# Biblbrox/ViT-Spectre-Experiments

Hardware: AMD Instinct MI355X
Metric: images/sec training, Spectre-ViT-S CIFAR-100 bs512 (higher is better)
Workload: dtype bf16; 1 GPU; Spectre-ViT-Small (E512 H16 F768 L4 P4 N65, 100 classes, dropout 0.001), fft mixer, train step fwd+CE+bwd+AdamW, bs 512/GPU; mixer=fft, global_batch=512, parallelism=dp1

## Files before the change

### include/spv.h

```cpp
#ifndef SPV_H
#define SPV_H

#include <stdint.h>

#ifdef __cplusplus
extern "C" {
#endif

#define SPV_F32 0
#define SPV_BF16 1

#define SPV_ABI_VERSION 1

int spv_version(void);
enum {
    SPV_PATH_GEMM_STRIP = 0,
    SPV_PATH_GEMM_STRIP_ACC = 1,
    SPV_PATH_GEMM_TN = 2,
    SPV_PATH_TAIL_LC = 3,
    SPV_PATH_TAIL_UP = 4,
    SPV_PATH_TAIL_LN = 5,
    SPV_PATH_FNET_MFMA = 6,
    SPV_PATH_GATHER_LDS = 7,
    SPV_PATH_GEMM_TN_WIDE = 9,
// ... 142 lines not shown
typedef struct spv_step_ctl {
    double a, b;
    float clip_coef;
    int apply;
    float grad_norm;
    int sched_step;
    int skipped;
    int reserved[7];
} spv_step_ctl;
#define SPV_CTL_SCHEDULE 1
#define SPV_CTL_CLIP 2
#define SPV_CTL_SKIP_NONFINITE 4

int spv_grad_sumsq(const void* table, const int* chunk_tensor, const int* chunk_off, const int* sizes, int nchunks, double* partials,
                   void* stream);

int spv_step_control(const double* partials, int npartials, float* const* step_ptrs, int nsteps, spv_step_ctl* ctl, int flags,
                     int warmup_steps, int total_steps, double eta_min, float max_norm, void* stream);

int spv_adamw_multi_ctl(const void* table, const int* chunk_tensor, const int* chunk_off, const int* sizes, int nchunks, double base_lr,
                        float beta1, float beta2, float one_minus_beta1, float one_minus_beta2, float eps, float weight_decay,
                        const float* step_dev, const spv_step_ctl* ctl, void* stream);

int spv_fwht(const void* x, void* y, const void* residual, int rows, int n_in, int n, int n_out, int mode, int repeat,
             float scale, int dtype, void* stream);

int spv_patchify(const float* img, void* out, int batch, int chans, int height, int width, int patch, int ld,
                 int transposed, int out_dtype, void* stream);
int spv_patchify_u8(const unsigned char* img_hwc, const float* mean, const float* inv_std, void* out, int batch, int chans,
                    int height, int width, int patch, int ld, int transposed, int out_dtype, void* stream);
int spv_embed_posbias(const float* pos, const float* bias, const float* cls, float* out, int patches, int embed, void* stream);
int spv_embed_cls_rows(const float* cls, const float* pos, void* tokens, int batch, int tokens_per_image, int embed,
                       int dtype, void* stream);
int spv_spectral_fold(const float* proj_w, const float* freq_h, const float* freq_w, float* w_full, int embed,
                      int chans, int patch, void* stream);
int spv_spectral_fold_bf16(const float* proj_w, const float* freq_h, const float* freq_w, float* w_full, void* w_full_bf16, int embed,
                           int chans, int patch, void* stream);
int spv_spectral_fold_bwd(const float* dw_full, const float* proj_w, const float* freq_h, const float* freq_w,
                          float* dproj_w, float* dfreq_h, float* dfreq_w, float* scratch, int embed, int chans,
                          int patch, void* stream);
int spv_dropout(const void* x, void* y, int64_t n, float p, uint64_t seed, int dtype, void* stream);
int spv_embed_bwd_groups(int batch);
int spv_embed_bwd(const void* g, const void* gcls, void* dtok, float* partials, float* dpos, float* dbias, float* dcls, int batch,
                  int tokens, int embed, float p_drop, uint64_t seed, int dtype, void* stream);

int spv_attention_fwd(const void* qkv, void* ctx, void* probs, int seqs, int len, int heads, int head_dim, int dtype,
                      float p_drop, uint64_t seed, void* stream);
int spv_attention_bwd(const void* dctx, const void* qkv, const void* probs, void* dscores, void* dqkv, int seqs, int len,
                      int heads, int head_dim, int dtype, float p_drop, uint64_t seed, void* stream);
int spv_attention_row0_fwd(const void* q0, const void* k, const void* v, int ldkv, void* ctx0, float* probs, int batch, int len,
                           int heads, int head_dim, int dtype, float p_drop, uint64_t seed, void* stream);
int spv_attention_row0_bwd(const void* dctx0, const void* q0, const void* k, const void* v, int ldkv, const float* probs, void* dq0,
                           void* dk, void* dv, int ldd, int batch, int len, int heads, int head_dim, int dtype, float p_drop,
                           uint64_t seed, void* stream);

int spv_gelu_fwd(const void* x, void* y, int64_t n, int dtype, void* stream);
int spv_gelu_bwd(const void* dy, const void* x, void* dx, int64_t n, int dtype, void* stream);
int spv_colsum(const void* x, float* out, float* partials, int rows, int n, int dtype, void* stream);
int spv_axpby(const void* x, const void* y, void* out, float a, float b, int64_t n, int dtype, void* stream);

int spv_small_sl_supported(int rows, int n, int k);
int64_t spv_small_sl_partial_floats(int rows, int n);
int spv_small_sl_fwd(const void* xa, int64_t lda, const void* xb, int64_t ldb, const float* W, const float* bias,
                     const float* gamma, const float* beta, float* out, float* h, float* xs, float* mean, float* rstd,
                     int rows, int n, int k, int dtype, void* stream);
int spv_small_sl_bwd(const float* dout, const float* h, const float* xs, const float* mean, const float* rstd,
// ... 67 lines not shown
```

### vit-spectre-experiments_amd/csrc/spv_patch.hip

```cpp
#define SPV_USES_SEED
#include "spv_common.h"

namespace {

__device__ __forceinline__ void st_any(void* base, size_t off, int bf, float v) {
    if (bf) static_cast<bf16_t*>(base)[off] = f2bf(v);
    else static_cast<float*>(base)[off] = v;
}
__device__ __forceinline__ float ld_any(const void* base, size_t off, int bf) {
    return bf ? bf2f(static_cast<const bf16_t*>(base)[off]) : static_cast<const float*>(base)[off];
}

__global__ __launch_bounds__(256) void patchify_kernel(const float* __restrict__ img, void* __restrict__ out, int B, int C, int H,
                                                       int W, int P, int ld, int transposed, int bf) {
    const int nH = H / P, nW = W / P, Np = nH * nW, K = C * P * P;
    const int64_t rows = (int64_t)B * Np;
    const int64_t total = transposed == 1 ? (int64_t)K * ld : (transposed == 2 ? (int64_t)B * (Np + 1) * ld : rows * ld);
    for (int64_t e = (int64_t)blockIdx.x * blockDim.x + threadIdx.x; e < total; e += (int64_t)gridDim.x * blockDim.x) {
        int64_t row;
        int k;
        if (transposed == 1) { k = (int)(e / ld); row = e % ld; }
        else { row = e / ld; k = (int)(e % ld); }
        if (transposed == 2) {
            const int64_t b2 = row / (Np + 1);
            const int t2 = (int)(row % (Np + 1));
            row = t2 == 0 ? rows : b2 * Np + t2 - 1;
        }
        float v = 0.0f;
        if (row < rows && k < K) {
            const int b = (int)(row / Np), n = (int)(row % Np);
            const int ih = n / nW, iw = n % nW;
            const int c = k / (P * P), p = (k / P) % P, q = k % P;
            v = img[(((size_t)b * C + c) * H + ih * P + p) * W + iw * P + q];
        }
// ... 185 lines not shown
                               batch, chans, height, width, patch, ld, transposed == 2);
        else
            hipLaunchKernelGGL((patchify_vec4_kernel<float>), dim3(ew_blocks(vecs)), dim3(256), 0, static_cast<hipStream_t>(stream), img, (float*)out,
                               batch, chans, height, width, patch, ld, transposed == 2);
        SPV_LAUNCH_CHECK("spv_patchify(vec4)");
        return 0;
    }
    hipLaunchKernelGGL(patchify_kernel, dim3(ew_blocks(total)), dim3(256), 0, static_cast<hipStream_t>(stream), img, out, batch,
                       chans, height, width, patch, ld, transposed, out_dtype == SPV_BF16);
    SPV_LAUNCH_CHECK("spv_patchify");
    return 0;
}

extern "C" int spv_patchify_u8(const unsigned char* img_hwc, const float* mean, const float* inv_std, void* out, int batch,
                               int chans, int height, int width, int patch, int ld, int transposed, int out_dtype, void* stream) {
    SPV_CHECK(batch > 0 && chans > 0 && patch > 0 && height >= patch && width >= patch, "spv_patchify_u8: bad shape");
    SPV_CHECK(out_dtype == SPV_F32 || out_dtype == SPV_BF16, "spv_patchify_u8: bad dtype");
    SPV_CHECK(mean != nullptr && inv_std != nullptr, "spv_patchify_u8: mean / inv_std missing");
    const int Np = (height / patch) * (width / patch), K = chans * patch * patch;
    const int64_t rows = (int64_t)batch * Np;
    SPV_CHECK(transposed >= 0 && transposed <= 2 && (transposed == 1 ? ld >= rows : ld >= K), "spv_patchify_u8: ld=%d too small", ld);
    const int64_t total = transposed == 1 ? (int64_t)K * ld : (transposed == 2 ? (int64_t)batch * (Np + 1) * ld : rows * ld);
    hipLaunchKernelGGL(patchify_u8_kernel, dim3(ew_blocks(total)), dim3(256), 0, static_cast<hipStream_t>(stream), img_hwc, mean,
                       inv_std, out, batch, chans, height, width, patch, ld, transposed, out_dtype == SPV_BF16);
    SPV_LAUNCH_CHECK("spv_patchify_u8");
    return 0;
}

extern "C" int spv_embed_posbias(const float* pos, const float* bias, const float* cls, float* out, int patches, int embed, void* stream) {
    SPV_CHECK(patches > 0 && embed > 0, "spv_embed_posbias: empty");
    hipLaunchKernelGGL(posbias_kernel, dim3(ew_blocks((int64_t)(patches + 1) * embed)), dim3(256), 0, static_cast<hipStream_t>(stream), pos,
                       bias, cls, out, patches, embed);
    SPV_LAUNCH_CHECK("spv_embed_posbias");
    return 0;
}

extern "C" int spv_embed_cls_rows(const float* cls, const float* pos, void* tokens, int batch, int tokens_per_image, int embed,
                                  int dtype, void* stream) {
    SPV_CHECK(batch > 0 && tokens_per_image > 0 && embed > 0, "spv_embed_cls_rows: empty");
    SPV_CHECK(dtype == SPV_F32 || dtype == SPV_BF16, "spv_embed_cls_rows: bad dtype");
    hipLaunchKernelGGL(cls_rows_kernel, dim3(ew_blocks((int64_t)batch * embed)), dim3(256), 0, static_cast<hipStream_t>(stream), cls,
                       pos, tokens, batch, tokens_per_image, embed, dtype == SPV_BF16);
    SPV_LAUNCH_CHECK("spv_embed_cls_rows");
    return 0;
}

constexpr int EB_GS = 16, EB_HB = 8;
template <typename T>
__global__ __launch_bounds__(256) void embed_bwd_rows_kernel(const T* __restrict__ g, const T* __restrict__ gcls, T* __restrict__ dtok,
                                                            float* __restrict__ partials, int B, int TE, int E, float p, uint64_t seed) {
    const int v = blockIdx.x * 256 + threadIdx.x;
    if (v * 8 >= TE) return;
    const int col = v * 8;
    const int b0 = blockIdx.y * EB_GS;
    const float inv_keep = 1.0f / (1.0f - p);
    const uint64_t sd = live_seed(seed);
    float acc[8];
#pragma unroll
    for (int u = 0; u < 8; ++u) acc[u] = 0.0f;
    const bool cls_row = gcls != nullptr && col < E;
    if constexpr (sizeof(T) == 2) {
        typedef unsigned raw4 __attribute__((ext_vector_type(4)));
        for (int h0 = 0; h0 < EB_GS; h0 += EB_HB) {
            raw4 xr[EB_HB], cr[EB_HB];
#pragma unroll
            for (int s = 0; s < EB_HB; ++s) xr[s] = *reinterpret_cast<const raw4*>(g + (size_t)min(b0 + h0 + s, B - 1) * TE + col);
// ... 192 lines not shown
```

### vit-spectre-experiments_amd/spectre_vit/_native.py

```python
import ctypes
import os

import torch

_HERE = os.path.dirname(os.path.abspath(__file__))
LIB_PATH = os.environ.get("SPV_LIB_PATH") or os.path.join(os.path.dirname(_HERE), "lib", "libspv_hip.so")

c_vp, c_i, c_i64, c_u64, c_f, c_d = ctypes.c_void_p, ctypes.c_int, ctypes.c_int64, ctypes.c_uint64, ctypes.c_float, ctypes.c_double

PATH = dict(gemm_strip=0, gemm_strip_acc=1, gemm_tn=2, tail_lc=3, tail_up=4, tail_ln=5, fnet_mfma=6, gather_lds=7, gemm_tn_wide=9,
            gemm_tn_batch=10, gemm_strip_pool=11, permut_row0=12, gemm_rows=13,
            spectrum=14, conv_fwd=15, conv_dgrad=16, conv_wgrad=17, token_pool=18, token_unpool=19, attn_row0_fwd=20, attn_row0_bwd=21, augment=22, teacher_view=23)

SIGNATURES = {
    "spv_version": [],
    "spv_last_error": [],
    "spv_path_count": [c_i],
    "spv_cast": [c_vp, c_i, c_vp, c_i, c_i64, c_vp],
    "spv_cast_transpose": [c_vp, c_i, c_vp, c_i, c_i, c_i, c_i, c_i, c_i, c_i, c_vp],
    "spv_weight_shadows": [c_vp, c_vp, c_vp, c_i, c_i, c_i, c_i, c_vp],
    "spv_weight_shadows_multi": [c_vp, c_vp, c_vp, c_vp, c_i, c_i, c_vp],
    "spv_gemm_nt": [c_vp, c_vp, c_vp, c_vp, c_i, c_i, c_i, c_i, c_i, c_i, c_i, c_i, c_i, c_i, c_vp, c_vp],
    "spv_gemm_nt_grouped_rows": [c_vp, c_vp, c_vp, c_vp, c_vp, c_i, c_i, c_i, c_i, c_i, c_i, c_i, c_i, c_i, c_i, c_i, c_vp],
    "spv_gemm_nt_grouped_rows_drop": [c_vp, c_vp, c_vp, c_vp, c_vp, c_i, c_i, c_i, c_i, c_i, c_i, c_i, c_i, c_i, c_i, c_i, c_f, c_u64, c_vp],
# ... 22 lines not shown
    "spv_haar_ln_bwd": [c_vp, c_vp, c_vp, c_vp, c_vp, c_vp, c_vp, c_vp, c_vp, c_i, c_i, c_i, c_vp],
    "spv_embed_bwd_groups": [c_i],
    "spv_embed_bwd": [c_vp, c_vp, c_vp, c_vp, c_vp, c_vp, c_vp, c_i, c_i, c_i, c_f, c_u64, c_i, c_vp],
    "spv_fold_multi": [c_vp, c_i, c_vp],
    "spv_gemm_tn_fold": [c_vp, c_vp, c_vp, c_i, c_i, c_i, c_i, c_i, c_i, c_i, c_i, c_i, c_vp, c_vp, c_i, c_vp],
    "spv_gemm_tn_batch": [c_vp, c_i, c_i, c_i, c_vp, c_vp, c_i, c_vp],
    "spv_gemm_tn_batch_part": [c_vp, c_i, c_i, c_i, c_vp, c_vp, c_i, c_i, c_vp],
    "spv_small_sl_supported": [c_i, c_i, c_i],
    "spv_small_sl_partial_floats": [c_i, c_i],
    "spv_small_sl_fwd": [c_vp, c_i64, c_vp, c_i64, c_vp, c_vp, c_vp, c_vp, c_vp, c_vp, c_vp, c_vp, c_vp, c_i, c_i, c_i, c_i, c_vp],
    "spv_small_sl_bwd": [c_vp] * 15 + [c_i, c_i, c_i, c_i, c_vp],
    "spv_cross_entropy_workspace_floats": [],
    "spv_cross_entropy_fwd": [c_vp, c_vp, c_vp, c_vp, c_vp, c_i, c_i, c_vp],
    "spv_cross_entropy_bwd": [c_vp, c_vp, c_vp, c_vp, c_vp, c_i, c_i, c_vp],
    "spv_permut_gather_fwd": [c_vp, c_vp, c_vp, c_vp, c_i, c_i, c_i, c_i, c_i, c_vp],
    "spv_gemm_nt_pool_bwd": [c_vp, c_vp, c_vp, c_vp, c_i, c_i, c_i, c_i, c_i, c_i, c_i, c_i, c_i, c_i, c_vp],
    "spv_permut_gather_bwd": [c_vp, c_vp, c_vp, c_i, c_i, c_i, c_i, c_vp],
    "spv_fnet_mix": [c_vp, c_vp, c_vp, c_vp, c_i, c_i, c_i, c_i, c_vp, c_vp],
    "spv_fnet_workspace_floats": [c_i, c_i, c_i],
    "spv_fnet_twiddle_floats": [c_i],
    "spv_fnet_make_twiddle": [c_vp, c_i, c_vp],
    "spv_fnet_ln_supported": [c_i, c_i, c_i],
    "spv_fnet_cls_supported": [c_i, c_i, c_i],
    "spv_fnet_cls_fwd": [c_vp, c_vp, c_vp, c_vp, c_vp, c_vp, c_vp, c_i, c_i, c_i, c_i, c_vp],
    "spv_fnet_cls_bwd": [c_vp, c_vp, c_vp, c_vp, c_vp, c_vp, c_vp, c_i, c_i, c_i, c_i, c_vp],
    "spv_fnet_ln_fwd": [c_vp, c_vp, c_vp, c_vp, c_vp, c_vp, c_vp, c_vp, c_i, c_i, c_i, c_i, c_vp],
    "spv_fnet_ln_bwd": [c_vp, c_vp, c_vp, c_vp, c_vp, c_vp, c_vp, c_vp, c_vp, c_vp, c_i, c_i, c_i, c_i, c_vp],
    "spv_rfft_real": [c_vp, c_vp, c_i, c_i, c_i, c_i, c_vp],
    "spv_haar_dwt": [c_vp, c_vp, c_i, c_i, c_i, c_i, c_i, c_i, c_i, c_vp, c_vp],
    "spv_patchify": [c_vp, c_vp, c_i, c_i, c_i, c_i, c_i, c_i, c_i, c_i, c_vp],
    "spv_patchify_u8": [c_vp, c_vp, c_vp, c_vp, c_i, c_i, c_i, c_i, c_i, c_i, c_i, c_i, c_vp],
    "spv_embed_posbias": [c_vp, c_vp, c_vp, c_vp, c_i, c_i, c_vp],
    "spv_embed_cls_rows": [c_vp, c_vp, c_vp, c_i, c_i, c_i, c_i, c_vp],
    "spv_spectral_fold": [c_vp, c_vp, c_vp, c_vp, c_i, c_i, c_i, c_vp],
    "spv_spectral_fold_bf16": [c_vp, c_vp, c_vp, c_vp, c_vp, c_i, c_i, c_i, c_vp],
    "spv_spectral_fold_bwd": [c_vp, c_vp, c_vp, c_vp, c_vp, c_vp, c_vp, c_vp, c_i, c_i, c_i, c_vp],
    "spv_dropout": [c_vp, c_vp, c_i64, c_f, c_u64, c_i, c_vp],
    "spv_attention_fwd": [c_vp, c_vp, c_vp, c_i, c_i, c_i, c_i, c_i, c_f, c_u64, c_vp],
    "spv_attention_bwd": [c_vp, c_vp, c_vp, c_vp, c_vp, c_i, c_i, c_i, c_i, c_i, c_f, c_u64, c_vp],
    "spv_attention_row0_fwd": [c_vp, c_vp, c_vp, c_i, c_vp, c_vp, c_i, c_i, c_i, c_i, c_i, c_f, c_u64, c_vp],
    "spv_attention_row0_bwd": [c_vp, c_vp, c_vp, c_vp, c_i, c_vp, c_vp, c_vp, c_vp, c_i, c_i, c_i, c_i, c_i, c_i, c_f, c_u64, c_vp],
    "spv_gelu_fwd": [c_vp, c_vp, c_i64, c_i, c_vp],
    "spv_gelu_bwd": [c_vp, c_vp, c_vp, c_i64, c_i, c_vp],
    "spv_colsum": [c_vp, c_vp, c_vp, c_i, c_i, c_i, c_vp],
    "spv_set_seed_device_ptr": [c_vp],
    "spv_seed_advance": [c_vp, c_vp],
    "spv_adamw_multi": [c_vp, c_vp, c_vp, c_vp, c_i, c_f, c_f, c_f, c_f, c_f, c_f, c_f, c_f, c_f, c_vp, c_vp],
    "spv_grad_sumsq": [c_vp, c_vp, c_vp, c_vp, c_i, c_vp, c_vp],
    "spv_step_control": [c_vp, c_i, c_vp, c_i, c_vp, c_i, c_i, c_i, c_d, c_f, c_vp],
    "spv_adamw_multi_ctl": [c_vp, c_vp, c_vp, c_vp, c_i, c_d, c_f, c_f, c_f, c_f, c_f, c_f, c_vp, c_vp, c_vp],
    "spv_fwht": [c_vp, c_vp, c_vp, c_i, c_i, c_i, c_i, c_i, c_i, c_f, c_i, c_vp],
    "spv_axpby": [c_vp, c_vp, c_vp, c_f, c_f, c_i64, c_i, c_vp],
    "spv_spectrum_floats": [c_i, c_i],
    "spv_spectrum_log1p": [c_vp, c_vp, c_i, c_i, c_i, c_i, c_i, c_vp],
    "spv_conv3x3_fwd": [c_vp, c_vp, c_vp, c_vp, c_vp, c_i, c_i, c_i, c_i, c_i, c_i, c_vp],
    "spv_conv3x3_dgrad": [c_vp, c_vp, c_vp, c_vp, c_i, c_i, c_i, c_i, c_i, c_i, c_vp],
    "spv_conv3x3_wgrad": [c_vp, c_vp, c_vp, c_vp, c_vp, c_vp, c_i, c_i, c_i, c_i, c_i, c_i, c_i, c_vp],
    "spv_token_pool_fwd": [c_vp, c_vp, c_i, c_i, c_i, c_i, c_i, c_i, c_vp],
    "spv_token_pool_bwd": [c_vp, c_i, c_vp, c_vp, c_i, c_i, c_i, c_i, c_i, c_vp],
    "spv_augment_params": [c_vp, c_i, c_i, c_i, c_i, c_vp, c_u64, c_u64, c_vp],
    "spv_augment_supported": [c_i, c_i, c_i],
    "spv_augment_u8": [c_vp, c_vp, c_vp, c_vp, c_vp, c_vp, c_i, c_i, c_i, c_i, c_i, c_vp],
    "spv_teacher_view_supported": [c_i, c_i, c_i, c_i],
    "spv_teacher_view_u8": [c_vp, c_vp, c_vp, c_vp, c_vp, c_i, c_i, c_i, c_i, c_i, c_i, c_i, c_vp],
    "spv_distill_loss_workspace_floats": [],
    "spv_distill_loss_fwd": [c_vp, c_vp, c_vp, c_vp, c_vp, c_vp, c_i, c_i, c_f, c_f, c_f, c_vp],
    "spv_distill_loss_bwd": [c_vp, c_vp, c_vp, c_vp, c_vp, c_vp, c_i, c_i, c_f, c_f, c_f, c_vp],
    "spv_eval_head_stats_words": [],
    "spv_eval_head": [c_vp, c_vp, c_vp, c_vp, c_vp, c_i, c_i, c_i, c_i, c_vp],
}
_RESTYPES = {"spv_last_error": ctypes.c_char_p, "spv_path_count": ctypes.c_longlong, "spv_rowop_partial_floats": c_i64, "spv_fnet_workspace_floats": c_i64,
             "spv_fnet_twiddle_floats": c_i64, "spv_tail_ln_partial_floats": c_i64, "spv_permut_table_words": c_i64, "spv_small_sl_partial_floats": c_i64,
             "spv_cross_entropy_workspace_floats": c_i64, "spv_distill_loss_workspace_floats": c_i64,
             "spv_eval_head_stats_words": c_i64}
_NO_STATUS = set(_RESTYPES) | {"spv_version", "spv_fnet_ln_supported", "spv_fnet_cls_supported", "spv_tail_ln_supported", "spv_tail_up_supported", "spv_small_sl_supported", "spv_tail_bwd_parts", "spv_embed_bwd_groups", "spv_haar_ln_supported", "spv_permut_pool_supported", "spv_spectrum_floats", "spv_augment_supported", "spv_teacher_view_supported"}

class FoldJob(ctypes.Structure):
    _fields_ = [("partials", c_vp), ("out", c_vp * 5), ("parts", c_i), ("nsum", c_i), ("n", c_i)]


class AugmentCfg(ctypes.Structure):
    _fields_ = [(n, c_f) for n in ("flip_p", "bright_lo", "bright_hi", "contrast_lo", "contrast_hi", "sat_lo", "sat_hi", "hue_lo", "hue_hi",
                                   "gray_p", "degrees", "blur_p", "sigma_lo", "sigma_hi", "erase_p", "scale_lo", "scale_hi", "ratio_lo",
                                   "ratio_hi")]


class TnProblem(ctypes.Structure):
    _fields_ = [("a", c_vp), ("b", c_vp), ("c", c_vp), ("m", c_i), ("n", c_i), ("lda", c_i), ("ldb", c_i), ("ldc", c_i), ("k", c_i)]


_lib = None
timer = None
hint = 0
_LAUNCHERS = {}


def load():
    global _lib
    if _lib is None:
        if not os.path.exists(LIB_PATH):
            raise RuntimeError(
                f"libspv_hip.so not found at {LIB_PATH}: build it with `python -c 'import __graft_entry__ as g; g.build()'` "
                "or `make -C vit-spectre-experiments_amd/csrc` (there is no CPU/PyTorch fallback for the Spectre-ViT kernels)")
        lib = ctypes.CDLL(LIB_PATH)
        for name, argtypes in SIGNATURES.items():
            fn = getattr(lib, name)
            fn.argtypes = argtypes
            fn.restype = _RESTYPES.get(name, c_i)
# ... 27 lines not shown
```

### vit-spectre-experiments_amd/spectre_vit/hip_ops.py

```python
from __future__ import annotations

import collections
import ctypes
import os
import warnings
import weakref
from typing import NamedTuple

import torch

from . import _native, shadows
from ._launch import _DT, BF16, F32, _dt, _p, _require_gpu, _stream
from .shadows import invalidate_weight_shadows
from .timing import KernelTimer, _timing, set_kernel_timer


_warned_fp16 = False


def compute_dtype(x: torch.Tensor) -> torch.dtype:
    global _warned_fp16
    if torch.is_autocast_enabled("cuda"):
        dt = torch.get_autocast_dtype("cuda")
        if dt == torch.float16:
# ... 596 lines not shown
        wf = torch.empty((E, chans * patch * patch), dtype=torch.float32, device=proj_w.device)
        if torch.is_autocast_enabled("cuda"):
            wb = torch.empty(wf.shape, dtype=torch.bfloat16, device=proj_w.device)
            _native.call("spv_spectral_fold_bf16", _p(proj_w), _p(fh), _p(fw), _p(wf), _p(wb), E, chans, patch, _stream())
            wf._spv_bf16 = wb
        else:
            _native.call("spv_spectral_fold", _p(proj_w), _p(fh), _p(fw), _p(wf), E, chans, patch, _stream())
        ctx.save_for_backward(proj_w, fh, fw)
        ctx.sinks = (_sink(proj_w), _sink(fh), _sink(fw))
        ctx.meta = (E, chans, patch)
        return wf

    @staticmethod
    def backward(ctx, dwf):
        proj_w, fh, fw = ctx.saved_tensors
        E, chans, patch = ctx.meta
        dwf = dwf.contiguous()
        dw = _grad_buf(ctx.sinks[0], proj_w.shape, proj_w.device)
        dfh = _grad_buf(ctx.sinks[1], fh.shape, fh.device)
        dfw = _grad_buf(ctx.sinks[2], fw.shape, fw.device)
        scratch = torch.empty_like(proj_w)
        _native.call("spv_spectral_fold_bwd", _p(dwf), _p(proj_w), _p(fh), _p(fw), _p(dw), _p(dfh), _p(dfw), _p(scratch), E,
                     chans, patch, _stream())
        return dw, dfh, dfw, None, None


class _EmbedKey:
    __slots__ = ("__weakref__",)


_cls_grad_stash = weakref.WeakKeyDictionary()


class PatchEmbedFn(torch.autograd.Function):

    @staticmethod
    def forward(ctx, img, w_full, bias, cls, pos, patch, dtype, norm=None, p_drop=0.0):
        _require_gpu(img, w_full)
        u8 = img.dtype == torch.uint8
        if u8:
            if norm is None:
                raise ValueError("uint8 images need the (mean, inv_std) normalisation tensors")
            B, H, W, C = img.shape
        else:
            B, C, H, W = img.shape
        E, K = w_full.shape
        Np = (H // patch) * (W // patch)
        T = Np + 1
        dev = img.device
        img = img.contiguous() if u8 else img.contiguous().float()
        _check_channels("patch embedding", E, K, dtype)
        st = _stream()
        patches = torch.empty((B * T, K), dtype=dtype, device=dev)
        if u8:
            _native.call("spv_patchify_u8", _p(img), _p(norm[0]), _p(norm[1]), _p(patches), B, C, H, W, patch, K, 2, _DT[dtype], st)
        else:
            _native.call("spv_patchify", _p(img), _p(patches), B, C, H, W, patch, K, 2, _DT[dtype], st)
        wc = w_full if dtype == torch.float32 else (getattr(w_full, "_spv_bf16", None) if dtype == torch.bfloat16 else None)
        if wc is None:
            wc = _raw_cast(w_full, dtype)
        posbias = torch.empty((T, E), dtype=torch.float32, device=dev)
        _native.call("spv_embed_posbias", _p(pos), _p(bias), _p(cls), _p(posbias), Np, E, st)
        tokens = torch.empty((B, T, E), dtype=dtype, device=dev)
        seed = _new_seed() if p_drop > 0.0 else 0
        _native.call("spv_gemm_nt_grouped_rows_drop", _p(patches), _p(wc), 0, _p(posbias), _p(tokens), B * T, E, K, K, K, E,
                     _DT[dtype], _DT[dtype], T, T, 0, float(p_drop), seed, st)
        ctx.save_for_backward(None if u8 else img, patches if (dtype == torch.bfloat16 or u8) else None)
        ctx.meta = (B, C, H, W, patch, E, K, Np, T, dtype, cls.shape, pos.shape, float(p_drop), seed)
        ctx.sinks = (_sink(bias), _sink(cls), _sink(pos))
        ctx.key = _EmbedKey()
        tokens._spv_embed_key = ctx.key
        return tokens

    @staticmethod
    def backward(ctx, dtok):
        img, patches = ctx.saved_tensors
        B, C, H, W, patch, E, K, Np, T, dtype, cls_shape, pos_shape, p_drop, seed = ctx.meta
        dev = dtok.device
        st = _stream()
        dtok = dtok.contiguous()
        early = start_held_wgrads()
        gcls = _cls_grad_stash.pop(ctx.key, None)
        if gcls is not None:
            gcls = gcls.to(dtok.dtype).contiguous()
        s_bias, s_cls, s_pos = ctx.sinks
        dpos_full = _grad_buf(s_pos, pos_shape, dev)
        dbias = _grad_buf(s_bias, (E,), dev)
        dcls = _grad_buf(s_cls, cls_shape, dev)
        part = torch.empty((_native.call("spv_embed_bwd_groups", B) * T * E,), dtype=torch.float32, device=dev)
        masked = torch.empty_like(dtok) if (gcls is not None or p_drop > 0.0) else None
        _native.call("spv_embed_bwd", _p(dtok), _p(gcls), _p(masked), _p(part), _p(dpos_full), _p(dbias), _p(dcls), B, T, E, p_drop, seed,
                     _dt(dtok), st)
        if masked is not None:
            dtok = masked
        if patches is not None and dtok.dtype == torch.bfloat16:
            dwf = _weight_grad(dtok.view(B * T, E), patches, B * T, E, K)
            if not early:
                join_side_stream()
            return None, dwf, dbias, dcls, dpos_full, None, None, None, None
# ... 781 lines not shown
```

### vit-spectre-experiments_amd/spectre_vit/timing.py

```python
from __future__ import annotations

import torch

from . import _native
from ._launch import BF16, F32

PEAK_TFLOPS = {BF16: 2500.0, F32: 157.3}
PEAK_HBM_GBS = 8000.0


def _es(dt):
    return 2 if dt == BF16 else 4


_WORK_MODELS = {
    "spv_small_sl_fwd": lambda i: ("head_fwd", i[2:5], i[5], "mfma", 2.0 * i[2] * i[3] * i[4]),
    "spv_small_sl_bwd": lambda i: ("head_bwd", i[0:3], i[3], "mfma", 4.0 * i[0] * i[1] * i[2]),
    "spv_cross_entropy_fwd": lambda i: ("cross_entropy_fwd", i[0:2], F32, "hbm", i[0] * i[1] * 4.0),
    "spv_cross_entropy_bwd": lambda i: ("cross_entropy_bwd", i[0:2], F32, "hbm", i[0] * i[1] * 8.0),
    "spv_distill_loss_fwd": lambda i: ("distill_loss_fwd", i[0:2], F32, "hbm", i[0] * i[1] * 8.0),
    "spv_distill_loss_bwd": lambda i: ("distill_loss_bwd", i[0:2], F32, "hbm", i[0] * i[1] * 12.0),
    "spv_teacher_view_u8": lambda i: ("teacher_view", (i[0], i[2], i[3], i[5]), i[6], "hbm",
                                      1.0 * i[0] * i[2] * (i[3] * i[3] + i[5] * i[5] * _es(i[6]))),
    "spv_gemm_nt": lambda i: ("gemm_acc" if i[8] else "gemm", i[0:3], i[6], "mfma", 2.0 * i[0] * i[1] * i[2]),
    "spv_gemm_nt_grouped_rows": lambda i: ("gemm_grouped_rows", i[0:3], i[6], "mfma", 2.0 * i[0] * i[1] * i[2]),
    "spv_gemm_nt_grouped_rows_drop": lambda i: ("gemm_grouped_rows", i[0:3], i[6], "mfma", 2.0 * i[0] * i[1] * i[2]),
    "spv_gemm_nt_pool_bwd": lambda i: ("gemm_pool_bwd", i[1:4], i[7], "mfma", 2.0 * i[1] * i[2] * i[3]),
    "spv_gemm_tn": lambda i: ("gemm_tn", i[0:3], BF16, "mfma", 2.0 * i[0] * i[1] * i[2]),
    "spv_gemm_tn_fold": lambda i: ("gemm_tn", i[0:3], BF16, "mfma", 2.0 * i[0] * i[1] * i[2]),
    "spv_gemm_tn_batch_part": lambda i: (("gemm_tn_batch", i[0:3], BF16, "mfma", float(i[-1])) if i[4] == 1 else
                                         ("splitk_reduce_batch", i[0:4], F32, "hbm", float(i[-1]))),
    "spv_embed_bwd": lambda i: ("embed_bwd", i[0:3], i[3], "hbm", 1.0 * i[0] * i[1] * i[2] * _es(i[3]) * (1 if (i[-2] >> 2) & 1 else 2)),
    "spv_fnet_cls_fwd": lambda i: ("fnet_cls_fwd", i[0:3], i[3], "hbm", 1.0 * i[0] * (i[1] + 1) * i[2] * _es(i[3])),
    "spv_fnet_cls_bwd": lambda i: ("fnet_cls_bwd", i[0:3], i[3], "hbm", 1.0 * i[0] * (i[1] + 1) * i[2] * _es(i[3])),
    "spv_permut_row0_fwd": lambda i: ("permut_row0_fwd", i[0:4], i[4], "hbm", 2.0 * i[0] * (i[2] + i[3]) * _es(i[4])),
    "spv_permut_row0_bwd": lambda i: ("permut_row0_bwd", i[0:4], i[4], "hbm", 1.0 * i[0] * (i[1] + i[2] + i[3]) * _es(i[4])),
    "spv_patchify": lambda i: ("patchify", i[0:5], i[7], "hbm",
                               1.0 * i[0] * i[1] * i[2] * i[3] * 4 + 1.0 * i[0] * ((i[2] // i[4]) * (i[3] // i[4]) + (i[6] == 2)) * i[5] * _es(i[7])),
    "spv_weight_shadows_multi": lambda i: ("weight_shadows_multi", i[0:1], i[1], "hbm", 2048.0 * i[0] * (4 + 2 * _es(i[1]))),
    "spv_spectre_tail_fwd": lambda i: ("tail_fwd", i[0:3], i[3], "hbm", i[0] * (2.0 * i[1] + i[2]) * _es(i[3])),
    "spv_spectre_tail_bwd": lambda i: ("tail_bwd" if not (i[-2] >> 7) & 1 else "tail_bwd_nodx", i[0:3], i[3], "hbm",
                                       i[0] * (3.0 * i[1] + (0 if (i[-2] >> 7) & 1 else i[2])) * _es(i[3])),
    "spv_spectre_tail_bwd_up": lambda i: ("tail_bwd_up", i[0:3], i[3], "hbm", i[0] * (3.0 * i[1] + 3.0 * i[2]) * _es(i[3])),
    "spv_spectre_tail_ln_fwd": lambda i: ("tail_ln_fwd", i[0:3], i[3], "hbm", i[0] * (4.0 * i[1] + i[2]) * _es(i[3])),
    "spv_spectre_tail_ln_bwd": lambda i: ("tail_ln_bwd", i[0:3], i[3], "hbm", i[0] * 6.0 * i[1] * _es(i[3])),
    "spv_add_layernorm_fwd": lambda i: ("addln_fwd", i[0:2], i[3], "hbm", 3.0 * i[0] * i[1] * _es(i[3])),
    "spv_add_layernorm_bwd": lambda i: ("addln_bwd", i[0:2], i[3], "hbm", (3.0 + (i[2] == 1)) * i[0] * i[1] * _es(i[3])),
    "spv_permut_gather_fwd": lambda i: ("gather_fwd", i[1:4], i[4], "hbm", i[1] * i[3] * (1.0 + i[2]) * _es(i[4])),
    "spv_permut_gather_bwd": lambda i: ("gather_bwd", i[0:3], i[3], "hbm", i[0] * i[2] * (1.0 + i[1]) * _es(i[3])),
    "spv_fnet_mix": lambda i: ("fnet_mix", i[0:3], i[3], "hbm", 2.0 * i[0] * i[1] * i[2] * _es(i[3])),
    "spv_fnet_ln_fwd": lambda i: ("fnet_ln_fwd", i[0:3], i[3], "hbm", 3.0 * i[0] * i[1] * i[2] * _es(i[3])),
    "spv_fnet_ln_bwd": lambda i: ("fnet_ln_bwd", i[0:3], i[3], "hbm", 3.0 * i[0] * i[1] * i[2] * _es(i[3])),
    "spv_haar_ln_fwd": lambda i: ("haar_ln_fwd", i[0:2], i[2], "hbm", 2.0 * i[0] * i[1] * _es(i[2])),
    "spv_haar_ln_bwd": lambda i: ("haar_ln_bwd", i[0:2], i[2], "hbm", 3.0 * i[0] * i[1] * _es(i[2])),
    "spv_haar_dwt": lambda i: ("haar_dwt", i[0:3], i[6], "hbm", 2.0 * i[0] * i[1] * i[2] * _es(i[6])),
    "spv_adamw_multi": lambda i: ("adamw_multi", i[0:1], F32, "hbm", 7.0 * 4 * 2048 * i[0]),
    "spv_grad_sumsq": lambda i: ("grad_sumsq", i[0:1], F32, "hbm", 4.0 * 2048 * i[0]),
    "spv_step_control": lambda i: ("step_control", i[0:2], F32, "hbm", 8.0 * i[0] + 64),
    "spv_adamw_multi_ctl": lambda i: ("adamw_multi_ctl", i[0:1], F32, "hbm", 7.0 * 4 * 2048 * i[0]),
    "spv_weight_shadows": lambda i: ("weight_shadows", i[0:2], i[3], "hbm", i[0] * i[1] * (4.0 + 2 * _es(i[3]))),
    "spv_dropout": lambda i: ("dropout", i[0:1], i[1], "hbm", 2.0 * i[0] * _es(i[1])),
    "spv_axpby": lambda i: ("axpby", i[0:1], i[1], "hbm", 3.0 * i[0] * _es(i[1])),
    "spv_colsum": lambda i: ("colsum", i[0:2], i[2], "hbm", 1.0 * i[0] * i[1] * _es(i[2])),
    "spv_cast": lambda i: ("cast", i[2:3], i[1], "hbm", 1.0 * i[2] * (_es(i[0]) + _es(i[1]))),
}


class KernelTimer:
    def __init__(self):
        self.records = []
        self.empties = []
# ... 69 lines not shown
```

Before: 321,300 images/sec.

## Fuse patchify, pos/bias add, and patch-embed GEMM into one MFMA kernel

Adds a single embed forward kernel that reads fp32 image pixels directly, packs them to bf16 MFMA operands in registers, multiplies by the bf16 projection weight, adds position/bias (or cls for token 0), applies dropout and writes bf16 tokens. It optionally writes the patches buffer for backward. This replaces three launches (patchify, posbias, grouped GEMM) and the intermediate patches/posbias round trips through memory. The fused path only covers patch 4, 3 channels, fp32 input and bf16 output, so other configurations keep the old path.

```diff
diff --git a/include/spv.h b/include/spv.h
--- a/include/spv.h
+++ b/include/spv.h
@@ -198,6 +198,10 @@
 int spv_embed_posbias(const float* pos, const float* bias, const float* cls, float* out, int patches, int embed, void* stream);
 int spv_embed_cls_rows(const float* cls, const float* pos, void* tokens, int batch, int tokens_per_image, int embed,
                        int dtype, void* stream);
+int spv_embed_fwd_supported(int chans, int height, int width, int patch, int embed, int in_dtype, int out_dtype);
+int spv_embed_fwd(const float* img, const void* w_bf16, const float* pos, const float* bias, const float* cls, void* tokens,
+                  void* patches, int batch, int chans, int height, int width, int patch, int embed, int in_dtype, int out_dtype,
+                  float p_drop, uint64_t seed, void* stream);
 int spv_spectral_fold(const float* proj_w, const float* freq_h, const float* freq_w, float* w_full, int embed,
                       int chans, int patch, void* stream);
 int spv_spectral_fold_bf16(const float* proj_w, const float* freq_h, const float* freq_w, float* w_full, void* w_full_bf16, int embed,
diff --git a/vit-spectre-experiments_amd/csrc/spv_embed_core.h b/vit-spectre-experiments_amd/csrc/spv_embed_core.h
--- /dev/null
+++ b/vit-spectre-experiments_amd/csrc/spv_embed_core.h
@@ -0,0 +1,44 @@
+#pragma once
+#include <stdint.h>
+
+#if defined(__HIPCC__)
+#define SPV_EHD __host__ __device__ __forceinline__
+#else
+#define SPV_EHD inline
+#endif
+
+constexpr int EMBED_P = 4;
+constexpr int EMBED_PP = 16;
+constexpr int EMBED_ROWS = 32;
+constexpr int EMBED_WAVE_COLS = 32;
+constexpr int EMBED_WG_COLS = 256;
+
+SPV_EHD void embed_share(int64_t total, int parts, int i, int64_t& beg, int64_t& end) {
+    const int64_t base = total / parts, rem = total % parts;
+    beg = (int64_t)i * base + (i < rem ? i : rem);
+    end = beg + base + (i < rem ? 1 : 0);
+}
+
+SPV_EHD void embed_unit(int g, int G, int col_ranges, int64_t rows, int& col_range, int64_t& rbeg, int64_t& rend) {
+    col_range = g % col_ranges;
+    embed_share(rows, G / col_ranges, g / col_ranges, rbeg, rend);
+}
+
+SPV_EHD void embed_row_bt(int64_t row, int T, int& b, int& t) {
+    b = (int)(row / T);
+    t = (int)(row - (int64_t)b * T);
+}
+SPV_EHD void embed_bt_advance(int& b, int& t, int T, int step) {
+    t += step;
+    while (t >= T) { t -= T; ++b; }
+}
+
+SPV_EHD unsigned embed_magic(int d) { return (unsigned)((1ull << 32) / (unsigned)d + 1u); }
+SPV_EHD int embed_div(int n, unsigned magic) { return (int)(((uint64_t)(unsigned)n * magic) >> 32); }
+
+SPV_EHD int64_t embed_img_offset(int b, int t, int k, int C, int H, int W, int nW, unsigned nw_magic) {
+    const int n = t - 1;
+    const int ih = embed_div(n, nw_magic), iw = n - ih * nW;
+    const int c = k >> 4, py = (k >> 2) & 3, px = k & 3;
+    return (((int64_t)b * C + c) * H + ih * EMBED_P + py) * W + iw * EMBED_P + px;
+}
diff --git a/vit-spectre-experiments_amd/csrc/spv_patch.hip b/vit-spectre-experiments_amd/csrc/spv_patch.hip
--- a/vit-spectre-experiments_amd/csrc/spv_patch.hip
+++ b/vit-spectre-experiments_amd/csrc/spv_patch.hip
@@ -1,5 +1,8 @@
 #define SPV_USES_SEED
 #include "spv_common.h"
+#include "spv_embed_core.h"
+
+#include <type_traits>
 
 namespace {
 
@@ -251,6 +254,158 @@
     hipLaunchKernelGGL(posbias_kernel, dim3(ew_blocks((int64_t)(patches + 1) * embed)), dim3(256), 0, static_cast<hipStream_t>(stream), pos,
                        bias, cls, out, patches, embed);
     SPV_LAUNCH_CHECK("spv_embed_posbias");
+    return 0;
+}
+
+constexpr int EF_WAVES = 8, EF_SLD = EMBED_WAVE_COLS + 4, EF_STAGE = 16 * EF_SLD + EMBED_ROWS;
+constexpr int EF_KS = 3;
+constexpr int EF_MAX_WGS = 256;
+typedef unsigned u32x4 __attribute__((ext_vector_type(4)));
+
+__device__ __forceinline__ void store16(void* dst, u32x4 o) { *reinterpret_cast<u32x4*>(dst) = o; }
+
+__global__ __launch_bounds__(EF_WAVES * 64) void embed_fwd_kernel(const float* __restrict__ img, const bf16_t* __restrict__ w,
+                                                                  const float* __restrict__ pos, const float* __restrict__ bias,
+                                                                  const float* __restrict__ cls, bf16_t* __restrict__ tokens,
+                                                                  bf16_t* __restrict__ patches, int B, int C, int H, int W, int E, int T,
+                                                                  int nW, unsigned nw_magic, int col_ranges, float p, uint64_t seed) {
+    __shared__ __attribute__((aligned(16))) float lds[EF_WAVES * EF_STAGE];
+    const int lane = threadIdx.x & 63, wave = threadIdx.x >> 6;
+    const int frow = lane & 31, fh = lane >> 5;
+    const int lr = lane >> 2, c8 = lane & 3;
+    float* stage = lds + wave * EF_STAGE;
+    unsigned* keys = reinterpret_cast<unsigned*>(stage + 16 * EF_SLD);
+    const int64_t R = (int64_t)B * T;
+    int cr;
+    int64_t rbeg, rend;
+    embed_unit(blockIdx.x, gridDim.x, col_ranges, R, cr, rbeg, rend);
+    if (rbeg >= rend) return;
+    const int cw = cr * EMBED_WG_COLS + wave * EMBED_WAVE_COLS;
+    const int K = EF_KS * EMBED_PP;
+
+    bf16x8 bfr[EF_KS];
+#pragma unroll
+    for (int ks = 0; ks < EF_KS; ++ks) bfr[ks] = *reinterpret_cast<const bf16x8*>(w + (size_t)(cw + frow) * K + ks * EMBED_PP + fh * 8);
+
+    const bool drop = p > 0.0f;
+    const uint64_t sd = drop ? live_seed(seed) : 0;
+    const float inv_keep = 1.0f / (1.0f - p);
+    const bool save = patches != nullptr && cr == 0 && wave < EF_KS;
+
+    auto load_a = [&](int b0, int t0, int step, float4 (&a)[2 * EF_KS], bool& zero) __attribute__((always_inline)) {
+        int b = b0, t = t0;
+        embed_bt_advance(b, t, T, step);
+        zero = t == 0;
+        const int tt = max(t, 1);
+#pragma unroll
+        for (int ks = 0; ks < EF_KS; ++ks) {
+            a[2 * ks] = *reinterpret_cast<const float4*>(img + embed_img_offset(b, tt, ks * EMBED_PP + fh * 8, C, H, W, nW, nw_magic));
+            a[2 * ks + 1] = *reinterpret_cast<const float4*>(img + embed_img_offset(b, tt, ks * EMBED_PP + fh * 8 + 4, C, H, W, nW, nw_magic));
+        }
+    };
+
+    int b0, t0;
+    embed_row_bt(rbeg, T, b0, t0);
+    float4 a[2 * EF_KS];
+    bool zero;
+    load_a(b0, t0, min(frow, (int)(R - 1 - rbeg)), a, zero);
+
+    auto block = [&](int64_t row0, auto full_tag) __attribute__((always_inline)) {
+        constexpr bool FULL = decltype(full_tag)::value;
+        const int last = (int)(R - 1 - row0);
+        bf16x8 af[EF_KS];
+        u32x4 q[EF_KS];
+#pragma unroll
+        for (int ks = 0; ks < EF_KS; ++ks) {
+            const float4 lo = a[2 * ks], hi = a[2 * ks + 1];
+            q[ks] = u32x4{pack_bf16x2(lo.x, lo.y), pack_bf16x2(lo.z, lo.w), pack_bf16x2(hi.x, hi.y), pack_bf16x2(hi.z, hi.w)};
+            if (zero) q[ks] = u32x4{0u, 0u, 0u, 0u};
+            af[ks] = __builtin_bit_cast(bf16x8, q[ks]);
+        }
+        if (save && (FULL || row0 + frow < rend))
+            store16(patches + (size_t)(row0 + frow) * K + wave * EMBED_PP + fh * 8, wave == 0 ? q[0] : (wave == 1 ? q[1] : q[2]));
+
+        float pb[2][8];
+#pragma unroll
+        for (int h = 0; h < 2; ++h) {
+            int b = b0, t = t0;
+            embed_bt_advance(b, t, T, min(16 * h + lr, last));
+            const float* p0 = pos + (size_t)t * E + cw + c8 * 8;
+            const float* p1 = (t == 0 ? cls : bias) + cw + c8 * 8;
+            const float4 x0 = *reinterpret_cast<const float4*>(p0), x1 = *reinterpret_cast<const float4*>(p0 + 4);
+            const float4 y0 = *reinterpret_cast<const float4*>(p1), y1 = *reinterpret_cast<const float4*>(p1 + 4);
+            pb[h][0] = x0.x + y0.x; pb[h][1] = x0.y + y0.y; pb[h][2] = x0.z + y0.z; pb[h][3] = x0.w + y0.w;
+            pb[h][4] = x1.x + y1.x; pb[h][5] = x1.y + y1.y; pb[h][6] = x1.z + y1.z; pb[h][7] = x1.w + y1.w;
+        }
+        load_a(b0, t0, min(EMBED_ROWS + frow, last), a, zero);
+
+        f32x16 acc;
+#pragma unroll
+        for (int r = 0; r < 16; ++r) acc[r] = 0.0f;
+#pragma unroll
+        for (int ks = 0; ks < EF_KS; ++ks) acc = __builtin_amdgcn_mfma_f32_32x32x16_bf16(af[ks], bfr[ks], acc, 0, 0, 0);
+
+        if (drop) keys[frow] = dropout_row_key(sd, (uint64_t)((row0 + min(frow, last)) * E + cw) >> 12);
+
+#pragma unroll
+        for (int h = 0; h < 2; ++h) {
+            if (!FULL && row0 + 16 * h >= rend) break;
+#pragma unroll
+            for (int r = 0; r < 8; ++r) stage[((r & 3) + 8 * (r >> 2) + 4 * fh) * EF_SLD + frow] = acc[8 * h + r];
+            __builtin_amdgcn_fence(__ATOMIC_RELEASE, "wavefront");
+            const float4 lo = *reinterpret_cast<const float4*>(stage + lr * EF_SLD + c8 * 8);
+            const float4 hi = *reinterpret_cast<const float4*>(stage + lr * EF_SLD + c8 * 8 + 4);
+            const unsigned key = drop ? keys[16 * h + lr] : 0u;
+            __builtin_amdgcn_fence(__ATOMIC_RELEASE, "wavefront");
+            float v[8] = {lo.x, lo.y, lo.z, lo.w, hi.x, hi.y, hi.z, hi.w};
+#pragma unroll
+            for (int u = 0; u < 8; ++u) v[u] += pb[h][u];
+            const int64_t row = row0 + 16 * h + lr;
+            const size_t fi = (size_t)row * E + cw + c8 * 8;
+            if (drop) {
+                const unsigned c0 = (unsigned)(fi & 4095);
+#pragma unroll
+                for (int u = 0; u < 8; ++u) v[u] *= dropout_scale(key, c0 + u, p, inv_keep);
+            }
+            const u32x4 o = {pack_bf16x2(v[0], v[1]), pack_bf16x2(v[2], v[3]), pack_bf16x2(v[4], v[5]), pack_bf16x2(v[6], v[7])};
+            if (FULL || row < rend) store16(tokens + fi, o);
+        }
+        embed_bt_advance(b0, t0, T, EMBED_ROWS);
+    };
+    int64_t row0 = rbeg;
+    if (row0 + EMBED_ROWS <= rend) {
+        block(row0, std::true_type{});
+        for (row0 += EMBED_ROWS; row0 + EMBED_ROWS <= rend; row0 += EMBED_ROWS) block(row0, std::true_type{});
+    }
+    if (row0 < rend) block(row0, std::false_type{});
+}
+
+extern "C" int spv_embed_fwd_supported(int chans, int height, int width, int patch, int embed, int in_dtype, int out_dtype) {
+    if (patch != EMBED_P || chans != EF_KS || height < EMBED_P || width < EMBED_P || width % 4 != 0) return 0;
+    if (embed <= 0 || embed % EMBED_WG_COLS != 0 || in_dtype != SPV_F32 || out_dtype != SPV_BF16) return 0;
+    const int64_t nW = width / EMBED_P, Np = (int64_t)(height / EMBED_P) * nW;
+    return Np * nW < (1ll << 32) ? 1 : 0;
+}
+
+extern "C" int spv_embed_fwd(const float* img, const void* w_bf16, const float* pos, const float* bias, const float* cls, void* tokens,
+                             void* patches, int batch, int chans, int height, int width, int patch, int embed, int in_dtype, int out_dtype,
+                             float p_drop, uint64_t seed, void* stream) {
+    SPV_CHECK(spv_embed_fwd_supported(chans, height, width, patch, embed, in_dtype, out_dtype),
+              "spv_embed_fwd: unsupported shape C=%d H=%d W=%d patch=%d E=%d dtypes %d -> %d (see spv_embed_fwd_supported)", chans, height,
+              width, patch, embed, in_dtype, out_dtype);
+    SPV_CHECK(batch > 0 && p_drop >= 0.0f && p_drop < 1.0f, "spv_embed_fwd: batch=%d p_drop=%f", batch, p_drop);
+    SPV_CHECK(img && w_bf16 && pos && bias && cls && tokens, "spv_embed_fwd: null pointer");
+    SPV_CHECK((((uintptr_t)img | (uintptr_t)w_bf16 | (uintptr_t)pos | (uintptr_t)bias | (uintptr_t)cls | (uintptr_t)tokens | (uintptr_t)patches) & 15) == 0,
+              "spv_embed_fwd: pointers must be 16-byte aligned");
+    const int nW = width / EMBED_P, T = (height / EMBED_P) * nW + 1;
+    const int64_t rows = (int64_t)batch * T;
+    SPV_CHECK(rows < (1ll << 31), "spv_embed_fwd: %lld token rows", (long long)rows);
+    const int col_ranges = embed / EMBED_WG_COLS;
+    const int workers = (int)std::max<int64_t>(1, std::min<int64_t>(EF_MAX_WGS / col_ranges, (rows + EMBED_ROWS - 1) / EMBED_ROWS));
+    hipLaunchKernelGGL(embed_fwd_kernel, dim3(workers * col_ranges), dim3(EF_WAVES * 64), 0, static_cast<hipStream_t>(stream), img,
+                       static_cast<const bf16_t*>(w_bf16), pos, bias, cls, static_cast<bf16_t*>(tokens), static_cast<bf16_t*>(patches), batch,
+                       chans, height, width, embed, T, nW, embed_magic(nW), col_ranges, p_drop, seed);
+    SPV_LAUNCH_CHECK("spv_embed_fwd");
     return 0;
 }
 
diff --git a/vit-spectre-experiments_amd/spectre_vit/_native.py b/vit-spectre-experiments_amd/spectre_vit/_native.py
--- a/vit-spectre-experiments_amd/spectre_vit/_native.py
+++ b/vit-spectre-experiments_amd/spectre_vit/_native.py
@@ -78,6 +78,8 @@
     "spv_patchify_u8": [c_vp, c_vp, c_vp, c_vp, c_i, c_i, c_i, c_i, c_i, c_i, c_i, c_i, c_vp],
     "spv_embed_posbias": [c_vp, c_vp, c_vp, c_vp, c_i, c_i, c_vp],
     "spv_embed_cls_rows": [c_vp, c_vp, c_vp, c_i, c_i, c_i, c_i, c_vp],
+    "spv_embed_fwd_supported": [c_i, c_i, c_i, c_i, c_i, c_i, c_i],
+    "spv_embed_fwd": [c_vp, c_vp, c_vp, c_vp, c_vp, c_vp, c_vp, c_i, c_i, c_i, c_i, c_i, c_i, c_i, c_i, c_f, c_u64, c_vp],
     "spv_spectral_fold": [c_vp, c_vp, c_vp, c_vp, c_i, c_i, c_i, c_vp],
     "spv_spectral_fold_bf16": [c_vp, c_vp, c_vp, c_vp, c_vp, c_i, c_i, c_i, c_vp],
     "spv_spectral_fold_bwd": [c_vp, c_vp, c_vp, c_vp, c_vp, c_vp, c_vp, c_vp, c_i, c_i, c_i, c_vp],
@@ -119,7 +121,7 @@
              "spv_fnet_twiddle_floats": c_i64, "spv_tail_ln_partial_floats": c_i64, "spv_permut_table_words": c_i64, "spv_small_sl_partial_floats": c_i64,
              "spv_cross_entropy_workspace_floats": c_i64, "spv_distill_loss_workspace_floats": c_i64,
              "spv_eval_head_stats_words": c_i64}
-_NO_STATUS = set(_RESTYPES) | {"spv_version", "spv_fnet_ln_supported", "spv_fnet_cls_supported", "spv_tail_ln_supported", "spv_tail_up_supported", "spv_small_sl_supported", "spv_tail_bwd_parts", "spv_embed_bwd_groups", "spv_haar_ln_supported", "spv_permut_pool_supported", "spv_spectrum_floats", "spv_augment_supported", "spv_teacher_view_supported"}
+_NO_STATUS = set(_RESTYPES) | {"spv_version", "spv_fnet_ln_supported", "spv_fnet_cls_supported", "spv_tail_ln_supported", "spv_tail_up_supported", "spv_small_sl_supported", "spv_tail_bwd_parts", "spv_embed_bwd_groups", "spv_embed_fwd_supported", "spv_haar_ln_supported", "spv_permut_pool_supported", "spv_spectrum_floats", "spv_augment_supported", "spv_teacher_view_supported"}
 
 class FoldJob(ctypes.Structure):
     _fields_ = [("partials", c_vp), ("out", c_vp * 5), ("parts", c_i), ("nsum", c_i), ("n", c_i)]
diff --git a/vit-spectre-experiments_amd/spectre_vit/hip_ops.py b/vit-spectre-experiments_amd/spectre_vit/hip_ops.py
--- a/vit-spectre-experiments_amd/spectre_vit/hip_ops.py
+++ b/vit-spectre-experiments_amd/spectre_vit/hip_ops.py
@@ -652,6 +652,9 @@
 _cls_grad_stash = weakref.WeakKeyDictionary()
 
 
+EMBED_FUSED = True
+
+
 class PatchEmbedFn(torch.autograd.Function):
 
     @staticmethod
@@ -671,20 +674,28 @@
         img = img.contiguous() if u8 else img.contiguous().float()
         _check_channels("patch embedding", E, K, dtype)
         st = _stream()
-        patches = torch.empty((B * T, K), dtype=dtype, device=dev)
-        if u8:
-            _native.call("spv_patchify_u8", _p(img), _p(norm[0]), _p(norm[1]), _p(patches), B, C, H, W, patch, K, 2, _DT[dtype], st)
-        else:
-            _native.call("spv_patchify", _p(img), _p(patches), B, C, H, W, patch, K, 2, _DT[dtype], st)
         wc = w_full if dtype == torch.float32 else (getattr(w_full, "_spv_bf16", None) if dtype == torch.bfloat16 else None)
         if wc is None:
             wc = _raw_cast(w_full, dtype)
-        posbias = torch.empty((T, E), dtype=torch.float32, device=dev)
-        _native.call("spv_embed_posbias", _p(pos), _p(bias), _p(cls), _p(posbias), Np, E, st)
         tokens = torch.empty((B, T, E), dtype=dtype, device=dev)
         seed = _new_seed() if p_drop > 0.0 else 0
-        _native.call("spv_gemm_nt_grouped_rows_drop", _p(patches), _p(wc), 0, _p(posbias), _p(tokens), B * T, E, K, K, K, E,
-                     _DT[dtype], _DT[dtype], T, T, 0, float(p_drop), seed, st)
+        fused = (EMBED_FUSED and not u8 and dtype == torch.bfloat16
+                 and _native.call("spv_embed_fwd_supported", C, H, W, patch, E, _DT[torch.float32], _DT[dtype]) == 1
+                 and all(t.data_ptr() % 16 == 0 for t in (img, wc, pos, bias, cls)))
+        if fused:
+            patches = torch.empty((B * T, K), dtype=dtype, device=dev) if any(ctx.needs_input_grad) else None
+            _native.call("spv_embed_fwd", _p(img), _p(wc), _p(pos), _p(bias), _p(cls), _p(tokens), _p(patches), B, C, H, W, patch, E,
+                         _DT[torch.float32], _DT[dtype], float(p_drop), seed, st)
+        else:
+            patches = torch.empty((B * T, K), dtype=dtype, device=dev)
+            if u8:
+                _native.call("spv_patchify_u8", _p(img), _p(norm[0]), _p(norm[1]), _p(patches), B, C, H, W, patch, K, 2, _DT[dtype], st)
+            else:
+                _native.call("spv_patchify", _p(img), _p(patches), B, C, H, W, patch, K, 2, _DT[dtype], st)
+            posbias = torch.empty((T, E), dtype=torch.float32, device=dev)
+            _native.call("spv_embed_posbias", _p(pos), _p(bias), _p(cls), _p(posbias), Np, E, st)
+            _native.call("spv_gemm_nt_grouped_rows_drop", _p(patches), _p(wc), 0, _p(posbias), _p(tokens), B * T, E, K, K, K, E,
+                         _DT[dtype], _DT[dtype], T, T, 0, float(p_drop), seed, st)
         ctx.save_for_backward(None if u8 else img, patches if (dtype == torch.bfloat16 or u8) else None)
         ctx.meta = (B, C, H, W, patch, E, K, Np, T, dtype, cls.shape, pos.shape, float(p_drop), seed)
         ctx.sinks = (_sink(bias), _sink(cls), _sink(pos))
diff --git a/vit-spectre-experiments_amd/spectre_vit/timing.py b/vit-spectre-experiments_amd/spectre_vit/timing.py
--- a/vit-spectre-experiments_amd/spectre_vit/timing.py
+++ b/vit-spectre-experiments_amd/spectre_vit/timing.py
@@ -11,6 +11,12 @@
 
 def _es(dt):
     return 2 if dt == BF16 else 4
+
+
+def _embed_fwd_bytes(i):
+    B, C, H, W, P, E = i[0:6]
+    T, K = (H // P) * (W // P) + 1, C * P * P
+    return 1.0 * B * C * H * W * 4 + (0 if (i[-2] >> 6) & 1 else B * T * K * 2) + B * T * E * 2 + T * E * 4
 
 
 _WORK_MODELS = {
@@ -37,6 +43,7 @@
     "spv_permut_row0_bwd": lambda i: ("permut_row0_bwd", i[0:4], i[4], "hbm", 1.0 * i[0] * (i[1] + i[2] + i[3]) * _es(i[4])),
     "spv_patchify": lambda i: ("patchify", i[0:5], i[7], "hbm",
                                1.0 * i[0] * i[1] * i[2] * i[3] * 4 + 1.0 * i[0] * ((i[2] // i[4]) * (i[3] // i[4]) + (i[6] == 2)) * i[5] * _es(i[7])),
+    "spv_embed_fwd": lambda i: ("embed_fwd", i[0:6], i[7], "hbm", _embed_fwd_bytes(i)),
     "spv_weight_shadows_multi": lambda i: ("weight_shadows_multi", i[0:1], i[1], "hbm", 2048.0 * i[0] * (4 + 2 * _es(i[1]))),
     "spv_spectre_tail_fwd": lambda i: ("tail_fwd", i[0:3], i[3], "hbm", i[0] * (2.0 * i[1] + i[2]) * _es(i[3])),
     "spv_spectre_tail_bwd": lambda i: ("tail_bwd" if not (i[-2] >> 7) & 1 else "tail_bwd_nodx", i[0:3], i[3], "hbm",
```

Measured after the change: 323,500 images/sec, median of 6. About the same (+0.7%).
